# ototoi/pbrt-r3

Measured on AMD Instinct MI355X. Metric: Mrays/s, higher is better.
Workload: dtype f32

## Files before the change

### pbrt-r3_amd/csrc/pt_kernels.hip

```cpp
#include <hip/hip_runtime.h>
#include <cstdlib>
#include "pt_device.h"
#include "pt_device_math.h"
#include "pt_bxdf.h"
#include "pt_sphere.h"
#include "pt_quadric.h"
#include "pt_texture.h"
#include <type_traits>
#include "pt_lobes.h"
#include "pt_kernels.h"
#include "../../include/pbrtgpu.h"

#if PT_QUADRIC
#define PT_KERNEL __global__
namespace ptq {
#else
#define PT_KERNEL extern "C" __global__
#endif

#ifndef PT_SHADE_PF_DEEP
#define PT_SHADE_PF_DEEP 0
#endif
#ifndef PT_LOBES_IN_LDS
#define PT_LOBES_IN_LDS 1
// ... 1859 lines not shown
    const float span = cdf1 - cdf0;
    if (span > 0.0f) du /= span;
    *pdf = func_int > 0.0f ? func[idx] / func_int : 0.0f;
    *off = idx;
    return ((float)idx + du) * (1.0f / (float)n);
}
PT_DEV float spherical_theta_dev(V3 v) { return pt_acosf(clampf(v.z, -1.0f, 1.0f)); }
PT_DEV float spherical_phi_dev(V3 v) { const float p = pt_atan2f(v.y, v.x); return p < 0.0f ? p + 2.0f * PT_PI : p; }
#define PT_INV_2PI (PT_INV_PI * 0.5f)
PT_DEV bool env_sample_li(const PtScene& sc, const PtEnvLight& e, V2 u, V3* li, V3* wi, float* pdf) {
    float pdf0, pdf1;
    uint32_t v, u_off;
    const float d1 = dist1d_sample_continuous(e.mfunc, e.mcdf, e.nv, e.m_int, u.y, &pdf1, &v);
    const float d0 = dist1d_sample_continuous(e.func + (size_t)v * e.nu, e.cdf + (size_t)v * (e.nu + 1u), e.nu, e.mfunc[v], u.x, &pdf0, &u_off);
    const float map_pdf = pdf0 * pdf1;
    if (map_pdf <= 0.0f) return false;
    const float theta = d1 * PT_PI, phi = d0 * 2.0f * PT_PI;
    float sin_t, cos_t, sin_p, cos_p;
    pt_sincosf(theta, &sin_t, &cos_t);
    pt_sincosf(phi, &sin_p, &cos_p);
    sin_t = clampf(sin_t, 0.0f, 1.0f);
    *wi = sph_vector(e.l2w, mk3(sin_t * cos_p, sin_t * sin_p, cos_t));
    *pdf = sin_t == 0.0f ? 0.0f : map_pdf / (2.0f * PT_PI * PT_PI * sin_t);
    *li = env_lookup0(sc, e, mk2(d0, d1));
    return true;
}
PT_DEV uint32_t dist_cell(float x, uint32_t n) { return !(x > 0.0f) ? 0u : (x >= (float)n ? n - 1u : min((uint32_t)x, n - 1u)); }
PT_DEV float env_pdf_li(const PtEnvLight& e, V3 w) {
    const V3 wl = sph_vector(e.w2l, w);
    const float theta = spherical_theta_dev(wl), phi = spherical_phi_dev(wl);
    float sin_t, cos_t;
    pt_sincosf(theta, &sin_t, &cos_t);
    sin_t = clampf(sin_t, 0.0f, 1.0f);
    if (sin_t == 0.0f) return 0.0f;
    const uint32_t iu = dist_cell(phi * PT_INV_2PI * (float)e.nu, e.nu), iv = dist_cell(theta * PT_INV_PI * (float)e.nv, e.nv);
    return e.func[(size_t)iv * e.nu + iu] / e.m_int / (2.0f * PT_PI * PT_PI * sin_t);
}
PT_DEV V3 env_le(const PtScene& sc, const PtEnvLight& e, V3 d) {
    const V3 w = normalize(sph_vector(e.w2l, d));
    return env_lookup0(sc, e, mk2(spherical_phi_dev(w) * PT_INV_2PI, spherical_theta_dev(w) * PT_INV_PI));
}
PT_DEV V3 env_le_all(const PtScene& sc, V3 d) {
    V3 r = mk3(0.0f, 0.0f, 0.0f);
    for (uint32_t k = 0; k < sc.n_envs; k++) r = r + env_le(sc, scene_envs(sc)[k], d);
    return r;
}
PT_DEV float spot_falloff(const PtDeltaLight& dl, V3 w) {
    const V3 wl = normalize(mk3(dl.w2l[0] * w.x + dl.w2l[1] * w.y + dl.w2l[2] * w.z, dl.w2l[3] * w.x + dl.w2l[4] * w.y + dl.w2l[5] * w.z,
                                dl.w2l[6] * w.x + dl.w2l[7] * w.y + dl.w2l[8] * w.z));
    const float cos_theta = wl.z;
    if (cos_theta < dl.cos_total_width) return 0.0f;
    if (cos_theta >= dl.cos_falloff_start) return 1.0f;
    const float delta = (cos_theta - dl.cos_total_width) / (dl.cos_falloff_start - dl.cos_total_width);
    return (delta * delta) * (delta * delta);
}
PT_DEV void delta_sample_li(const PtDeltaLight& dl, V3 ref_p, V3* li, V3* wi, float* pdf, V3* lp) {
    const V3 v = ld3(dl.v), sp = ld3(dl.spectrum);
    *pdf = 1.0f;
    if (dl.kind == PT_DELTA_DISTANT) {
        *wi = v;
        *li = sp;
        *lp = ref_p + v * (2.0f * dl.radius);
        return;
    }
    *wi = normalize(v - ref_p);
    const float d2 = distance_squared(v, ref_p);
    if (dl.kind == PT_DELTA_SPOT) *li = sp * (spot_falloff(dl, -*wi) / d2);
    else *li = sp / d2;
    *lp = v;
}
template <bool DELTA>
PT_DEV bool light_is_delta(const PtLight& l) { if constexpr (DELTA) return (l.mesh_flags & PT_LIGHT_DELTA) != 0; else return false; }
template <bool SPH, bool ENV, bool DELTA = ENV>
PT_DEV bool light_sample_kind(const PtScene& sc, const PtLight& l, V3 ref_p, V3 ref_pe, V3 ref_n, V2 u, V3* li, V3* wi, float* pdf, V3* lp, V3* lperr,
                              V3* ln) {
    if constexpr (ENV) {
        if (l.mesh_flags & PT_LIGHT_INFINITE) {
            const PtEnvLight& e = scene_envs(sc)[__float_as_uint(l.p0[0])];
            if (!env_sample_li(sc, e, u, li, wi, pdf)) return false;
            *lp = ref_p + *wi * (2.0f * e.radius);
            *lperr = mk3(0.0f, 0.0f, 0.0f); *ln = mk3(0.0f, 0.0f, 0.0f);
            return true;
        }
        if constexpr (DELTA) {
            if (l.mesh_flags & PT_LIGHT_DELTA) {
                delta_sample_li(scene_deltas(sc)[__float_as_uint(l.p0[0])], ref_p, li, wi, pdf, lp);
                *lperr = mk3(0.0f, 0.0f, 0.0f); *ln = mk3(0.0f, 0.0f, 0.0f);
                return true;
            }
        }
    }
    return light_sample_any<SPH>(sc, l, ref_p, ref_pe, ref_n, u, li, wi, pdf, lp, lperr, ln);
}

PT_DEV const float* grid_lookup(const PtLightGrid& g, V3 p) {
    if (g.single) return g.data;
    uint32_t pi[3];
    float pc[3] = {p.x, p.y, p.z};
    for (int i = 0; i < 3; i++) {
        float o = pc[i] - g.wb_min[i];
        if (g.wb_max[i] > g.wb_min[i]) o = o / (g.wb_max[i] - g.wb_min[i]);
        o = clampf(o, 0.0f, 1.0f);
        float f = o * (float)g.voxels[i];
        uint32_t v = f > 0.0f ? (uint32_t)f : 0u;
        if (v > g.voxels[i] - 1) v = g.voxels[i] - 1;
        pi[i] = v;
    }
    size_t vox = ((size_t)pi[2] * g.voxels[1] + pi[1]) * g.voxels[0] + pi[0];
    if (g.row_of) vox = (size_t)(uint32_t)g.row_of[vox];
    return g.data + vox * g.stride;
}
PT_DEV uint32_t sample_discrete(const float* tab, uint32_t n, float u, float* pdf) {
    uint32_t idx;
    float f_idx, func_int;
    if (n <= 3) {
        const float4* q = reinterpret_cast<const float4*>(tab);
        float4 a = q[0], b = q[1];
        auto get = [&](uint32_t i) -> float {
            float lo = i == 0 ? a.x : (i == 1 ? a.y : (i == 2 ? a.z : a.w));
            float hi = i == 4 ? b.x : (i == 5 ? b.y : (i == 6 ? b.z : b.w));
            return i < 4 ? lo : hi;
        };
        uint32_t first = 0, len = n + 1;
        while (len > 0) {
            uint32_t half = len >> 1, middle = first + half;
            if (get(n + middle) <= u) { first = middle + 1; len -= half + 1; }
            else len = half;
        }
        idx = first == 0 ? 0 : first - 1;
        if (idx > n - 1) idx = n - 1;
        f_idx = get(idx);
        func_int = get(2 * n + 1);
    } else {
        const float* cdf = tab + n;
        uint32_t first = 0, len = n + 1;
        while (len > 0) {
            uint32_t half = len >> 1, middle = first + half;
            if (cdf[middle] <= u) { first = middle + 1; len -= half + 1; }
            else len = half;
        }
        idx = first == 0 ? 0 : first - 1;
        if (idx > n - 1) idx = n - 1;
        f_idx = tab[idx];
        func_int = tab[2 * n + 1];
    }
    *pdf = func_int > 0.0f ? f_idx * (1.0f / (float)n) / func_int : 0.0f;
    return idx;
}

PT_KERNEL void __launch_bounds__(PT_BLOCK) k_nee_resolve(PtScene sc, PtPaths P, PtQueues Q) {
    const uint32_t n = Q.counts[PT_Q_NEE];
    for (uint32_t i = blockIdx.x * blockDim.x + threadIdx.x; i < n; i += gridDim.x * blockDim.x) {
        const uint32_t p = Q.nee[i];
        const uint32_t nee = P.nee[p];
        const float4 A = P.pendA[p];
        V3 ld = mk3(0.0f, 0.0f, 0.0f);
        if ((nee & PT_NEE_SHADOW) && P.occluded[p] == 0) ld = ld + mk3(A.x, A.y, A.z);
        if (nee & PT_NEE_PROBE) {
            const int32_t best = P.probe_rec[p];
            if (best >= 0 && (uint32_t)best == sc.lights[nee >> 8].tri_rec) { float4 B = P.pendB[p]; ld = ld + mk3(B.x, B.y, B.z); }
        }
        V3 ldn = ld / A.w;
        float4 pb = P.pbeta[p];
        float4 L = P.L[p];
        V3 add = mk3(pb.x, pb.y, pb.z) * ldn;
        L.x += add.x; L.y += add.y; L.z += add.z;
        P.L[p] = L;
    }
}
PT_KERNEL void __launch_bounds__(PT_BLOCK) k_nee_resolve_env(PtScene sc, PtPaths P, PtQueues Q) {
    const uint32_t n = Q.counts[PT_Q_NEE];
    for (uint32_t i = blockIdx.x * blockDim.x + threadIdx.x; i < n; i += gridDim.x * blockDim.x) {
        const uint32_t p = Q.nee[i];
        const uint32_t nee = P.nee[p];
        const float4 A = P.pendA[p];
        V3 ld = mk3(0.0f, 0.0f, 0.0f);
        if ((nee & PT_NEE_SHADOW) && P.occluded[p] == 0) ld = ld + mk3(A.x, A.y, A.z);
        if (nee & PT_NEE_PROBE) {
            const int32_t best = P.probe_rec[p];
            const PtLight& lt = sc.lights[nee >> 8];
            const bool take = (lt.mesh_flags & PT_LIGHT_INFINITE) ? best < 0 : (best >= 0 && (uint32_t)best == lt.tri_rec);
            if (take) { float4 B = P.pendB[p]; ld = ld + mk3(B.x, B.y, B.z); }
        }
        V3 ldn = ld / A.w;
        float4 pb = P.pbeta[p];
        float4 L = P.L[p];
        V3 add = mk3(pb.x, pb.y, pb.z) * ldn;
        L.x += add.x; L.y += add.y; L.z += add.z;
        P.L[p] = L;
    }
}

PT_DEV uint32_t path_sort_bin(const PtScene& sc, const PtPaths& P, uint32_t p) {
    int32_t rec = P.hit_rec[p];
    if (rec < 0) return 0xffffffffu;
    uint32_t m1 = sc.tris[rec].flags >> PT_TRI_MATERIAL_SHIFT;
    return m1 == 0 ? (sc.n_instances ? PT_SORT_GENERAL0 : 0u) : sc.materials[m1 - 1].sort_bin;
}
PT_DEV uint32_t wave_bin_reserve(uint32_t* counters, uint32_t bin, bool valid) {
    uint32_t slot = 0;
    unsigned long long todo = __ballot(valid);
    const uint32_t lane = threadIdx.x & 63;
    while (todo) {
        int leader = __ffsll((long long)todo) - 1;
        uint32_t b0 = (uint32_t)__shfl((int)bin, leader, 64);
        unsigned long long same = __ballot(valid && bin == b0) & todo;
        uint32_t base = 0;
        if ((int)lane == leader) base = atomicAdd(&counters[b0], (uint32_t)__popcll(same));
        base = (uint32_t)__shfl((int)base, leader, 64);
        if (valid && bin == b0) slot = base + (uint32_t)__popcll(same & ((lane == 0) ? 0ull : (~0ull >> (64 - lane))));
        todo &= ~same;
    }
    return slot;
}
PT_DEV void sort_chunk(uint32_t n, uint32_t* lo, uint32_t* hi) {
    uint32_t chunk = (n + gridDim.x - 1) / gridDim.x;
    chunk = (chunk + 63u) & ~63u;
    *lo = min(n, blockIdx.x * chunk);
    *hi = min(n, *lo + chunk);
}
PT_KERNEL void __launch_bounds__(PT_BLOCK) k_sort_count(PtScene sc, PtPaths P, PtQueues Q) {
    __shared__ uint32_t s_cnt[PT_SORT_BINS];
    s_cnt[threadIdx.x] = 0;
    __syncthreads();
    uint32_t lo, hi;
    sort_chunk(Q.counts[PT_Q_CUR], &lo, &hi);
    for (uint32_t i = lo + threadIdx.x; i < ((hi + 63u) & ~63u); i += blockDim.x) {
        bool valid = i < hi;
        uint32_t bin = valid ? path_sort_bin(sc, P, Q.cur[i]) : 0xffffffffu;
        if (valid && Q.bin) Q.bin[i] = (uint16_t)bin;
        valid = valid && bin != 0xffffffffu;
        (void)wave_bin_reserve(s_cnt, valid ? bin : 0u, valid);
    }
    __syncthreads();
    uint32_t c = s_cnt[threadIdx.x];
    if (c) atomicAdd(&Q.counts[PT_SORT_COUNT0 + threadIdx.x], c);
}
PT_KERNEL void k_sort_scan(PtQueues Q) {
    __shared__ uint32_t s[PT_SORT_BINS];
    const uint32_t t = threadIdx.x;
    uint32_t c = Q.counts[PT_SORT_COUNT0 + t];
    s[t] = c;
    __syncthreads();
    for (uint32_t d = 1; d < PT_SORT_BINS; d <<= 1) {
        uint32_t v = t >= d ? s[t - d] : 0u;
        __syncthreads();
        s[t] += v;
        __syncthreads();
    }
    uint32_t excl = s[t] - c;
    Q.counts[PT_SORT_CURSOR0 + t] = excl;
    Q.counts[PT_SORT_COUNT0 + t] = 0;
    if (t == PT_SORT_GENERAL0) Q.counts[PT_Q_MATTE_END] = excl;
    if (t == PT_SORT_TEX0) Q.counts[PT_Q_TEX_BEGIN] = excl;
    if (t == PT_SORT_BINS - 1) Q.counts[PT_Q_GENERAL_END] = s[t];
}
PT_KERNEL void __launch_bounds__(PT_BLOCK) k_sort_scatter(PtScene sc, PtPaths P, PtQueues Q) {
    __shared__ uint32_t s_cnt[PT_SORT_BINS];
    s_cnt[threadIdx.x] = 0;
    __syncthreads();
    uint32_t lo, hi;
    sort_chunk(Q.counts[PT_Q_CUR], &lo, &hi);
    const uint32_t hi_round = (hi + 63u) & ~63u;
    auto bin_of = [&](uint32_t i, uint32_t p) -> uint32_t {
        if (Q.bin) { const uint32_t b = Q.bin[i]; return b == 0xffffu ? 0xffffffffu : b; }
        return path_sort_bin(sc, P, p);
    };
    for (uint32_t i = lo + threadIdx.x; i < hi_round; i += blockDim.x) {
        bool valid = i < hi;
        uint32_t bin = valid ? bin_of(i, Q.bin ? 0u : Q.cur[i]) : 0xffffffffu;
        valid = valid && bin != 0xffffffffu;
        (void)wave_bin_reserve(s_cnt, valid ? bin : 0u, valid);
    }
    __syncthreads();
    {
        uint32_t c = s_cnt[threadIdx.x];
        s_cnt[threadIdx.x] = c ? atomicAdd(&Q.counts[PT_SORT_CURSOR0 + threadIdx.x], c) : 0u;
    }
    __syncthreads();
    for (uint32_t i = lo + threadIdx.x; i < hi_round; i += blockDim.x) {
        bool valid = i < hi;
        uint32_t p = valid ? Q.cur[i] : 0u;
        uint32_t bin = valid ? bin_of(i, p) : 0xffffffffu;
        valid = valid && bin != 0xffffffffu;
        uint32_t pos = wave_bin_reserve(s_cnt, valid ? bin : 0u, valid);
        if (valid) Q.sorted[pos] = p;
    }
}

#ifndef PT_LOCAL_CHUNK
#define PT_LOCAL_CHUNK 4096u
#endif
PT_KERNEL void __launch_bounds__(PT_BLOCK) k_sort_local(PtScene sc, PtPaths P, PtQueues Q) {
    __shared__ uint32_t s_cnt[PT_SORT_BINS + 1];
    __shared__ uint32_t s_p[PT_LOCAL_CHUNK];
    __shared__ uint16_t s_b[PT_LOCAL_CHUNK];
    const uint32_t n = Q.counts[PT_Q_CUR];
    const uint32_t n_runs = (n + PT_LOCAL_CHUNK - 1u) / PT_LOCAL_CHUNK;
    for (uint32_t run = blockIdx.x; run < n_runs; run += gridDim.x) {
        const uint32_t lo = run * PT_LOCAL_CHUNK, len = min(PT_LOCAL_CHUNK, n - lo);
        for (uint32_t k = threadIdx.x; k <= PT_SORT_BINS; k += blockDim.x) s_cnt[k] = 0;
        __syncthreads();
        for (uint32_t i = threadIdx.x; i < len; i += blockDim.x) {
            const uint32_t p = Q.cur[lo + i];
            const uint32_t bin = path_sort_bin(sc, P, p);
            const uint32_t b = bin == 0xffffffffu ? PT_SORT_BINS : bin;
            s_p[i] = p; s_b[i] = (uint16_t)b;
            atomicAdd(&s_cnt[b], 1u);
        }
        __syncthreads();
        if (threadIdx.x == 0) {
            uint32_t acc = 0;
            for (uint32_t k = 0; k <= PT_SORT_BINS; k++) { const uint32_t c = s_cnt[k]; s_cnt[k] = acc; acc += c; }
        }
        __syncthreads();
        for (uint32_t i = threadIdx.x; i < len; i += blockDim.x) {
            const uint32_t pos = atomicAdd(&s_cnt[s_b[i]], 1u);
            Q.sorted[lo + pos] = s_p[i];
        }
        __syncthreads();
    }
}

#ifndef PT_SHADE_TICKET
#define PT_SHADE_TICKET 4
#endif
#ifndef PT_SHADE_FLUSH
#define PT_SHADE_FLUSH 4
// ... 103 lines not shown
            V3 c_n = n0, c_dpdu = dpdu0;
            textured_lobes(sc, mj, th, &tm, n, uv, &c_n, &c_dpdu, sh_dpdv, sh_dndu, sh_dndv);
            lm = &tm;
        }
        if (j == 0) eta0 = lm->bsdf_eta;
        if (lm->has_bsdf)
            for (uint32_t i = 0; i < lm->n_lobes && nl < PT_MIX_MAX_LOBES; i++) {
                mh->lobes[nl] = lm->lobes[i];
                mh->scales.lobe_leaf[nl] = j;
                nl++;
            }
        const uint32_t nc = mx.scales.n_chain[j];
        mh->scales.n_chain[j] = nc;
        for (uint32_t c = 0; c < nc; c++) {
            const uint32_t e = mx.chain[j][c], node = e & 0xffu, side = (e >> 8) & 1u;
            for (int q = 0; q < 3; q++) mh->scales.s[j][c][q] = ns[node][side][q];
        }
    }
    out->type = PT_MATERIAL_MIX;
    out->has_bsdf = 1; out->nonspecular = 0; out->spec_mask = 0; out->bsdf_eta = eta0;
    out->n_lobes = nl;
    for (uint32_t i = 0; i < nl; i++) {
        const uint32_t t = mh->lobes[i].type;
        if (!(t & kSpecular)) out->nonspecular++;
        if ((t & (kRefl | kSpecular)) == t) out->spec_mask |= 1u;
        if ((t & (kTrans | kSpecular)) == t) out->spec_mask |= 2u;
    }
}
PT_DEV void mix_hit(const PtScene& sc, int32_t material, const TexHit& th, PtMaterial* out, PtMixHit* mh, Surf& s) {
    const int32_t m0 = material_mix(sc, sc.materials[material]).leaf_material[0];
    const V3 n0 = s.sh_n, dpdu0 = s.sh_dpdu;
    uint32_t leaf0_done = 0;
    if (sc.materials[m0].textured) {
        textured_lobes(sc, m0, th, out, s.n, s.uv, &s.sh_n, &s.sh_dpdu, s.sh_dpdv, s.sh_dndu, s.sh_dndv);
        leaf0_done = 1;
    }
    mix_hit_lobes(sc, material, th, out, leaf0_done, mh, s.n, s.uv, n0, dpdu0, s.sh_dpdv, s.sh_dndu, s.sh_dndv);
}
PT_DEV uint32_t ray_sort_key(const PtScene& sc, V3 o, V3 d) {
    const float fx = (o.x - sc.wb_min[0]) * sc.cell_scale[0], fy = (o.y - sc.wb_min[1]) * sc.cell_scale[1], fz = (o.z - sc.wb_min[2]) * sc.cell_scale[2];
    const float top = (float)((1u << PT_SORT_CELL_BITS) - 1u);
    uint32_t cx = (uint32_t)fminf(fmaxf(fx, 0.0f), top), cy = (uint32_t)fminf(fmaxf(fy, 0.0f), top), cz = (uint32_t)fminf(fmaxf(fz, 0.0f), top);
    uint32_t m = 0;
#pragma unroll
    for (uint32_t b = 0; b < (uint32_t)PT_SORT_CELL_BITS; b++) m |= (((cx >> b) & 1u) | (((cy >> b) & 1u) << 1) | (((cz >> b) & 1u) << 2)) << (3u * b);
    return m | ((d.x < 0.0f ? 1u : 0u) | (d.y < 0.0f ? 2u : 0u) | (d.z < 0.0f ? 4u : 0u)) << (3u * PT_SORT_CELL_BITS);
}
#ifdef PT_PROFILE_SHADE
__device__ unsigned long long g_shade_prof[16];
#define PT_SHP(k) do { const unsigned long long t_now_ = (unsigned long long)__builtin_readcyclecounter(); shp_acc[k] += t_now_ - shp_last; shp_last = t_now_; } while (0)
#define PT_SHP_SYNC(k) do { asm volatile("s_waitcnt vmcnt(0)" ::: "memory"); PT_SHP(k); } while (0)
#else
#define PT_SHP(k) do { } while (0)
#define PT_SHP_SYNC(k) do { } while (0)
#endif
PT_DEV float opaque_zero() { float z = 0.0f; asm volatile("" : "+v"(z)); return z; }
template <bool GENERAL, bool SPH, bool TEX = false, bool INST = false, bool RES = false, int PART = 0, bool ENV = false, bool DELTA = false, bool MIX = false>
PT_DEV void shade_body(const PtScene& sc, const PtPaths& P, const PtQueues& Q, PtCounters* cnt, const uint32_t* list, uint32_t begin, uint32_t end,
                       uint32_t* ticket) {
    __shared__ unsigned long long s_vert;
    __shared__ float4 s_stage[PART == 2 ? 1 : 7][PT_BLOCK];
    __shared__ uint32_t s_pend[PT_SHADE_FLUSH][PT_BLOCK];
#if PT_LOBES_IN_LDS
    __shared__ uint32_t s_lobes[GENERAL ? PT_BLOCK / 64 : 1][PT_MAX_LOBES * (sizeof(PtLobe) / 4)];
#endif
    __shared__ uint32_t s_pkey[PT_SHADE_FLUSH][PT_BLOCK];
    if (threadIdx.x == 0) s_vert = 0;
#if PT_LIGHTS_IN_LDS
    __shared__ PtLight s_lights[PT_LIGHTS_IN_LDS];
    const bool lights_lds = sc.n_lights <= (uint32_t)PT_LIGHTS_IN_LDS && PART != 2;
    if (lights_lds) {
        const uint32_t nd = sc.n_lights * (uint32_t)(sizeof(PtLight) / 4);
        const uint32_t* src = reinterpret_cast<const uint32_t*>(sc.lights);
        uint32_t* dst = reinterpret_cast<uint32_t*>(s_lights);
        for (uint32_t k = threadIdx.x; k < nd; k += PT_BLOCK) dst[k] = src[k];
    }
#endif
    __syncthreads();
    uint32_t n_vert = 0;
    const uint32_t lane = threadIdx.x & 63;
    uint32_t chunk_left = 0, next_base = 0;
#ifdef PT_PROFILE_SHADE
    unsigned long long shp_acc[16] = {0, 0, 0, 0, 0, 0, 0, 0, 0, 0, 0, 0, 0, 0, 0, 0};
    unsigned long long shp_last = (unsigned long long)__builtin_readcyclecounter();
#endif
    uint32_t n_batch = 0, pend_want = 0;
    uint32_t pf_p = 0;
    int32_t pf_rec = -1;
    uint32_t pf_st = 0, pf_pk = 0;
    uint64_t pf_idx = 0;
    bool pf_valid = false;
    constexpr bool DEEP = PT_SHADE_PF_DEEP && !GENERAL && !SPH && !INST && PART == 0;
    float4 pf_ro = make_float4(0.0f, 0.0f, 0.0f, 0.0f), pf_rd = pf_ro, pf_beta = pf_ro, pf_ra = pf_ro, pf_rb = pf_ro, pf_rc = pf_ro;
    const unsigned long long below = (lane == 0) ? 0ull : (~0ull >> (64 - lane));
    auto flush_batch = [&]() {
        if (n_batch == 0) return;
        uint32_t tc = 0, tn = 0, ts = 0, tp = 0;
#pragma unroll
        for (uint32_t j = 0; j < PT_SHADE_FLUSH; j++) {
            if (j < n_batch) {
                const uint32_t e = pend_want >> (4u * j);
                tc += (uint32_t)__popcll(__ballot((e & 1u) != 0)); tn += (uint32_t)__popcll(__ballot((e & 2u) != 0));
                ts += (uint32_t)__popcll(__ballot((e & 4u) != 0)); tp += (uint32_t)__popcll(__ballot((e & 8u) != 0));
            }
        }
        uint32_t bc = 0, bn = 0, bs = 0, bp = 0;
        if (lane == 0) {
            if (tc) bc = atomicAdd(&Q.counts[PT_Q_NEXT], tc);
            if (tn) bn = atomicAdd(&Q.counts[PT_Q_NEE], tn);
            if (ts) bs = atomicAdd(&Q.counts[PT_Q_SHADOW], ts);
            if (tp) bp = atomicAdd(&Q.counts[PT_Q_PROBE], tp);
        }
        bc = (uint32_t)__builtin_amdgcn_readfirstlane((int)bc); bn = (uint32_t)__builtin_amdgcn_readfirstlane((int)bn);
        bs = (uint32_t)__builtin_amdgcn_readfirstlane((int)bs); bp = (uint32_t)__builtin_amdgcn_readfirstlane((int)bp);
#pragma unroll
        for (uint32_t j = 0; j < PT_SHADE_FLUSH; j++) {
            if (j < n_batch) {
                const uint32_t e = pend_want >> (4u * j), ep = s_pend[j][threadIdx.x];
                const unsigned long long mc = __ballot((e & 1u) != 0), mn = __ballot((e & 2u) != 0), ms = __ballot((e & 4u) != 0), mp = __ballot((e & 8u) != 0);
                if (e & 1u) Q.next[bc + (uint32_t)__popcll(mc & below)] = ep;
                if (e & 2u) Q.nee[bn + (uint32_t)__popcll(mn & below)] = ep;
                if (e & 4u) {
                    Q.shadow[bs + (uint32_t)__popcll(ms & below)] = ep;
                    if (Q.shadow_key) Q.shadow_key[bs + (uint32_t)__popcll(ms & below)] = s_pkey[j][threadIdx.x];
                }
                if (e & 8u) Q.probe[bp + (uint32_t)__popcll(mp & below)] = ep;
                bc += (uint32_t)__popcll(mc); bn += (uint32_t)__popcll(mn); bs += (uint32_t)__popcll(ms); bp += (uint32_t)__popcll(mp);
            }
        }
        n_batch = 0; pend_want = 0;
    };
    for (;;) {
        PT_SHP(11);
        if (chunk_left == 0) {
            uint32_t t0 = 0;
            if (lane == 0) t0 = atomicAdd(ticket, 64u * PT_SHADE_TICKET);
            next_base = begin + (uint32_t)__builtin_amdgcn_readfirstlane((int)t0);
            chunk_left = PT_SHADE_TICKET;
        }
        uint32_t base = next_base;
        next_base += 64u; chunk_left--;
        if (base >= end) break;
#ifdef PT_PROFILE_SHADE
        shp_acc[12]++;
#endif
        uint32_t item = base + lane;
        bool active = item < end;
        bool cont = false, want_nee = false, want_sh = false, want_pr = false;
        uint32_t p = 0;
        uint32_t wr = 0, o_nee = 0, o_state = 0;
        float4 o_ray_o = make_float4(0.0f, 0.0f, 0.0f, 0.0f), o_ray_d = o_ray_o, o_beta = o_ray_o;
        auto commit = [&]() {
            if constexpr (PART != 2) {
                if (wr & 4u) { P.sh_o[p] = s_stage[0][threadIdx.x]; P.sh_d[p] = s_stage[1][threadIdx.x]; }
                if (wr & 8u) { P.pr_o[p] = s_stage[2][threadIdx.x]; P.pr_d[p] = s_stage[3][threadIdx.x]; }
                if (wr & 16u) { P.pendA[p] = s_stage[4][threadIdx.x]; P.pendB[p] = s_stage[5][threadIdx.x]; P.pbeta[p] = s_stage[6][threadIdx.x]; P.nee[p] = o_nee; }
            }
            if (wr & 1u) P.ray_o[p] = o_ray_o;
            if (wr & 2u) { P.ray_d[p] = o_ray_d; P.beta[p] = o_beta; }
            if (wr & 32u) P.state[p] = o_state;
            wr = 0;
        };
#ifndef PT_DEFER_WIDE
#define PT_DEFER_WIDE 0
#endif
#ifndef PT_DEFER_SITES
#define PT_DEFER_SITES (PT_DEFER_WIDE ? 63 : 0)
#endif
#define PT_COMMIT_NOW(site) do { if constexpr ((TEX || INST) && !((PT_DEFER_SITES >> (site)) & 1)) commit(); } while (0)
        const bool had_pf = pf_valid;
        const uint32_t pf_p_now = pf_p;
        const int32_t pf_rec_now = pf_rec;
        const uint32_t pf_st_now = pf_st, pf_pk_now = pf_pk;
        const uint64_t pf_idx_now = pf_idx;
        const float4 pf_ro_now = pf_ro, pf_rd_now = pf_rd, pf_beta_now = pf_beta, pf_ra_now = pf_ra, pf_rb_now = pf_rb, pf_rc_now = pf_rc;
        pf_valid = chunk_left > 0;
        const bool pf_lane = pf_valid && next_base + lane < end;
        if (pf_lane) pf_p = list[next_base + lane];
        if (active) {
            p = had_pf ? pf_p_now : list[item];
            PT_SHP_SYNC(13);
            float4 ro4, rd4, beta4;
            if (DEEP && had_pf) { ro4 = pf_ro_now; rd4 = pf_rd_now; beta4 = pf_beta_now; }
            else { ro4 = P.ray_o[p]; rd4 = P.ray_d[p]; beta4 = P.beta[p]; }
            V3 ro = f4_3(ro4), rd = f4_3(rd4);
            int32_t rec = had_pf ? pf_rec_now : P.hit_rec[p];
            uint32_t st = had_pf ? pf_st_now : P.state[p];
            uint32_t dim = st & 0xffffu, bounces = (st >> 16) & 0xffu, flags = st >> 24;
            V3 beta = f4_3(beta4);
            float eta_scale = beta4.w;
            PT_SHP_SYNC(14);
            float4 rec_a = make_float4(0.0f, 0.0f, 0.0f, 0.0f), rec_b = rec_a, rec_c = rec_a;
            if (DEEP && had_pf) { rec_a = pf_ra_now; rec_b = pf_rb_now; rec_c = pf_rc_now; }
            else if (rec >= 0) {
                const float4* q = reinterpret_cast<const float4*>(sc.tris) + (size_t)(uint32_t)rec * 3;
                rec_a = q[0]; rec_b = q[1]; rec_c = q[2];
            }
            SamplerPre sm;
            sm.s.index = 0; sm.s.dim = dim; sm.s.px = 0; sm.s.py = 0; sm.dim0 = dim; sm.have = false;
            if (rec >= 0 && (int32_t)bounces < sc.max_depth) {
                sm.s.index = had_pf ? pf_idx_now : P.sobol_index[p];
                const uint32_t pk = had_pf ? pf_pk_now : P.pixel[p];
                sm.s.px = (int32_t)(pk & 0xffffu) + sc.film.sample_bounds[0];
                sm.s.py = (int32_t)(pk >> 16) + sc.film.sample_bounds[1];
                PT_SHP_SYNC(15);
                sm.begin(sc);
                PT_SHP_SYNC(10);
            }
            Surf s;
            float thit;
            bool found;
            if constexpr (INST) found = rec >= 0 && make_surf_inst<SPH>(sc, ro, rd, (uint32_t)rec, P.hit_inst[p], s, &thit);
            else found = rec >= 0 && make_surf_any_rec<SPH>(sc, ro, rd, (uint32_t)rec, rec_a, rec_b, rec_c, s, &thit);
            PT_SHP(0);
            if (pf_lane) {
                pf_rec = P.hit_rec[pf_p];
                pf_st = P.state[pf_p]; pf_idx = P.sobol_index[pf_p]; pf_pk = P.pixel[pf_p];
                if constexpr (DEEP) { pf_ro = P.ray_o[pf_p]; pf_rd = P.ray_d[pf_p]; pf_beta = P.beta[pf_p]; }
            }
            if constexpr (ENV && PART != 1) {
                if (rec < 0 && (bounces == 0 || (flags & PT_ST_SPECULAR))) {
                    float4 L = P.L[p];
                    for (uint32_t k = 0; k < sc.n_envs; k++) {
                        const V3 add = beta * env_le(sc, scene_envs(sc)[k], rd);
                        L.x += add.x; L.y += add.y; L.z += add.z;
                    }
                    P.L[p] = L;
                }
            }
            if (PART != 1 && found && (bounces == 0 || (flags & PT_ST_SPECULAR))) {
                int32_t li = s.light;
                if (li >= 0) {
                    V3 le = light_L(sc.lights[li], s.n, -rd);
                    float4 L = P.L[p];
                    V3 add = beta * le;
                    L.x += add.x; L.y += add.y; L.z += add.z;
                    P.L[p] = L;
                }
            }
            if (found && (int32_t)bounces < sc.max_depth) {
                bool no_bsdf = s.material < 0;
                PtMaterial tm;
                std::conditional_t<MIX, PtMixHit, PtNoMix> mh;
                bool use_tm = false;
                if constexpr (TEX) {
                    if (!no_bsdf && sc.materials[s.material].textured) {
                        TexHit th;
                        th.p = s.p; th.uv = s.uv;
                        RayDiffs rdf;
                        const bool has_diff = (flags & PT_ST_CAMERA) != 0;
                        if (has_diff) {
                            Sampler sl;
                            sl.index = P.sobol_index[p];
                            sl.dim = 2;
                            uint32_t pk2 = P.pixel[p];
                            sl.px = (int32_t)(pk2 & 0xffffu) + sc.film.sample_bounds[0];
                            sl.py = (int32_t)(pk2 >> 16) + sc.film.sample_bounds[1];
                            V2 u_lens = mk2(0.0f, 0.0f);
                            if (sc.cam.lens_radius > 0.0f) u_lens = sl.get_2d(sc);
                            float2 pf = P.p_film[p];
                            camera_differentials(sc, mk2(pf.x, pf.y), u_lens, ro, rd, rdf);
                        }
                        compute_differentials(th, s.p, s.n, s.dpdu, s.dpdv, has_diff, rdf);
                        if constexpr (MIX) {
                            if (sc.materials[s.material].mix1) mix_hit(sc, s.material, th, &tm, &mh, s);
                            else textured_lobes(sc, s.material, th, &tm, s.n, s.uv, &s.sh_n, &s.sh_dpdu, s.sh_dpdv, s.sh_dndu, s.sh_dndv);
                        } else
                        textured_lobes(sc, s.material, th, &tm, s.n, s.uv, &s.sh_n, &s.sh_dpdu, s.sh_dpdv, s.sh_dndu, s.sh_dndv);
                        use_tm = true;
                        no_bsdf = tm.has_bsdf == 0;
                    }
                }
                if constexpr (RES) {
                    if (!no_bsdf && sc.materials[s.material].textured) {
                        const float4* r = P.tex_res + (size_t)p * PT_TEX_RES_F4;
                        const float4 r0 = r[0], r1 = r[1], r2 = r[2], r3 = r[3], r4 = r[4], r5 = r[5], r6 = r[6], r7 = r[7], r8 = r[8];
                        PtMatParams mp = sc.mat_params[s.material];
                        mp.m.kd[0] = r0.x; mp.m.kd[1] = r0.y; mp.m.kd[2] = r0.z; mp.m.ks[0] = r0.w; mp.m.ks[1] = r1.x; mp.m.ks[2] = r1.y;
                        mp.m.kr[0] = r1.z; mp.m.kr[1] = r1.w; mp.m.kr[2] = r2.x; mp.m.kt[0] = r2.y; mp.m.kt[1] = r2.z; mp.m.kt[2] = r2.w;
                        mp.m.opacity[0] = r3.x; mp.m.opacity[1] = r3.y; mp.m.opacity[2] = r3.z; mp.m.sigma = r3.w;
                        mp.m.metal_eta[0] = r4.x; mp.m.metal_eta[1] = r4.y; mp.m.metal_eta[2] = r4.z; mp.m.metal_k[0] = r4.w; mp.m.metal_k[1] = r5.x; mp.m.metal_k[2] = r5.y;
                        mp.m.uroughness = r5.z; mp.m.vroughness = r5.w; mp.m.eta = r6.x;
                        build_lobes_call(mp.m, r6.y, r6.z, r6.w, tm);
                        s.sh_n = mk3(r7.x, r7.y, r7.z); s.sh_dpdu = mk3(r7.w, r8.x, r8.y);
                        use_tm = true;
                        no_bsdf = tm.has_bsdf == 0;
                    }
                }
                if constexpr (GENERAL) { if (!no_bsdf && !use_tm) no_bsdf = sc.materials[s.material].has_bsdf == 0; }
                if (no_bsdf) {
                    if constexpr (PART != 1) {
                        V3 no = offset_ray_origin(s.p, s.p_error, s.n, rd);
                        o_ray_o = make_float4(no.x, no.y, no.z, PT_INF); wr |= 1u;
                        cont = true; PT_COMMIT_NOW(0);
                    }
                } else {
                    if constexpr (PART != 1) n_vert++;
                    Bsdf b;
                    std::conditional_t<MIX, MBsdf, GBsdf> gb;
                    bool nonspecular;
                    float bsdf_eta = 1.0f;
                    if constexpr (GENERAL) {
                        const PtMaterial& m = use_tm ? tm : sc.materials[s.material];
                        gb.ns = s.sh_n; gb.ng = s.n;
                        gb.ss = normalize(s.sh_dpdu);
                        gb.ts = normalize(cross(gb.ns, gb.ss));
                        gb.lobes = m.lobes; gb.n_lobes = m.n_lobes;
                        if constexpr (MIX) {
                            gb.scales = nullptr;
                            if (sc.materials[s.material].mix1) {
                                if (use_tm) { gb.lobes = mh.lobes; gb.scales = &mh.scales; }
                                else { const PtMix& mx = material_mix(sc, sc.materials[s.material]); gb.lobes = mx.lobes; gb.n_lobes = mx.n_lobes; gb.scales = &mx.scales; }
                            }
                        }
#if PT_LOBES_IN_LDS
                        if constexpr (!INST && !TEX) {
                            const int32_t mat0 = __builtin_amdgcn_readfirstlane(s.material);
                            const unsigned long long here = __ballot(1);
                            if (__ballot(use_tm || s.material != mat0) == 0ull) {
                                const uint32_t nd = (uint32_t)__builtin_amdgcn_readfirstlane((int)m.n_lobes) * (uint32_t)(sizeof(PtLobe) / 4);
                                const uint32_t nact = (uint32_t)__popcll(here), rank = (uint32_t)__popcll(here & below);
                                const uint32_t* src = reinterpret_cast<const uint32_t*>(sc.materials[mat0].lobes);
                                uint32_t* dst = &s_lobes[threadIdx.x >> 6][0];
                                for (uint32_t k = rank; k < nd; k += nact) dst[k] = src[k];
                                __builtin_amdgcn_fence(__ATOMIC_RELEASE, "wavefront");
                                __builtin_amdgcn_wave_barrier();
                                __builtin_amdgcn_fence(__ATOMIC_ACQUIRE, "wavefront");
                                gb.lobes = reinterpret_cast<const PtLobe*>(dst);
                            }
                        }
#endif
                        nonspecular = m.nonspecular > 0;
                        bsdf_eta = m.bsdf_eta;
                    } else {
                        const PtMaterial& m = sc.materials[s.material];
                        b.ns = s.sh_n; b.ng = s.n;
                        b.ss = normalize(s.sh_dpdu);
                        b.ts = normalize(cross(b.ns, b.ss));
                        b.r = mk3(m.kd[0], m.kd[1], m.kd[2]);
                        b.n_lobes = is_black(b.r) ? 0 : 1;
                        b.oren = clampf(m.sigma, 0.0f, 90.0f) != 0.0f;
                        b.oa = m.oren_a; b.ob = m.oren_b;
                        nonspecular = b.n_lobes > 0;
                    }
                    const uint32_t kNoSpec = PT_BSDF_ALL & ~PT_BSDF_SPECULAR;
                    auto eval_f = [&](V3 wo_w, V3 wi_w) -> V3 {
                        if constexpr (MIX) return mbsdf_f(gb, wo_w, wi_w, kNoSpec);
                        else if constexpr (GENERAL) return gbsdf_f(gb, wo_w, wi_w, kNoSpec); else return bsdf_f(b, wo_w, wi_w);
                    };
                    auto eval_pdf = [&](V3 wo_w, V3 wi_w) -> float {
                        if constexpr (MIX) return mbsdf_pdf(gb, wo_w, wi_w, kNoSpec);
                        else if constexpr (GENERAL) return gbsdf_pdf(gb, wo_w, wi_w, kNoSpec); else return bsdf_pdf(b, wo_w, wi_w);
                    };
                    auto sample_bsdf = [&](V3 wo_w, V2 uu, uint32_t fl, V3* f_o, V3* wi_o, float* pdf_o, uint32_t* type_o) -> bool {
                        if constexpr (MIX) return mbsdf_sample_f(gb, wo_w, uu, fl, f_o, wi_o, pdf_o, type_o);
                        else if constexpr (GENERAL) return gbsdf_sample_f(gb, wo_w, uu, fl, f_o, wi_o, pdf_o, type_o);
                        else { *type_o = PT_BSDF_REFLECTION | PT_BSDF_DIFFUSE; return bsdf_sample_f(b, wo_w, uu, f_o, wi_o, pdf_o); }
                    };
                    PT_SHP(1);
                    if constexpr (PART == 2) {
                        if (nonspecular && sc.n_lights > 0) sm.s.dim += (P.nee[p] & PT_NEE_DIMS5) ? 5u : 1u;
                    }
                    if (PART != 2 && nonspecular && sc.n_lights > 0) {
                        const float* tab = grid_lookup(sc.grid, s.p);
                        float light_pdf;
                        uint32_t light_num = sample_discrete(tab, sc.n_lights, sm.get_1d(sc), &light_pdf);
                        PT_SHP(2);
                        if (light_pdf > 0.0f) {
                            V2 u_light = sm.get_2d(sc);
                            V2 u_scat = sm.get_2d(sc);
                            PT_SHP(3);
#if PT_LIGHTS_IN_LDS
                            const PtLight& lt = lights_lds ? s_lights[light_num] : sc.lights[light_num];
#else
                            const PtLight& lt = sc.lights[light_num];
#endif
                            uint32_t nee = (light_num << 8) | (PART == 1 ? PT_NEE_DIMS5 : 0u);
                            V3 A = mk3(0.0f, 0.0f, 0.0f), B = mk3(0.0f, 0.0f, 0.0f);
                            V3 li, wi, lp, lperr, ln;
                            float lpdf;
                            bool sampled;
                            if constexpr (ENV) sampled = light_sample_kind<SPH, true, DELTA>(sc, lt, s.p, s.p_error, s.n, u_light, &li, &wi, &lpdf, &lp, &lperr, &ln);
                            else sampled = light_sample_any<SPH>(sc, lt, s.p, s.p_error, s.n, u_light, &li, &wi, &lpdf, &lp, &lperr, &ln);
                            if (sampled) {
                                if (lpdf > 0.0f && !is_black(li)) {
                                    V3 f = eval_f(s.wo, wi) * abs_dot(wi, s.sh_n);
                                    float spdf = eval_pdf(s.wo, wi);
                                    if (!is_black(f)) {
                                        V3 origin = offset_ray_origin(s.p, s.p_error, s.n, lp - s.p);
                                        V3 target = offset_ray_origin(lp, lperr, ln, origin - lp);
                                        V3 sd = target - origin;
                                        s_stage[0][threadIdx.x] = make_float4(origin.x, origin.y, origin.z, 1.0f - PT_SHADOW_EPS);
                                        s_stage[1][threadIdx.x] = make_float4(sd.x, sd.y, sd.z, 0.0f);
                                        if (Q.shadow_key) s_pkey[n_batch][threadIdx.x] = ray_sort_key(sc, origin, sd);
                                        wr |= 4u; PT_COMMIT_NOW(1);
                                        if (light_is_delta<DELTA>(lt)) A = f * li / lpdf;
                                        else {
                                            float weight = power_heuristic(lpdf, spdf);
                                            A = f * li * (weight / lpdf);
                                        }
                                        nee |= PT_NEE_SHADOW;
                                    }
                                }
                            }
                            PT_SHP(4);
                            V3 f2, wi2;
                            float spdf2;
                            uint32_t type2;
                            if (!light_is_delta<DELTA>(lt) && sample_bsdf(s.wo, u_scat, kNoSpec, &f2, &wi2, &spdf2, &type2)) {
                                V3 f = f2 * abs_dot(wi2, s.sh_n);
                                if (!is_black(f) && spdf2 > 0.0f) {
                                    V3 po = offset_ray_origin(s.p, s.p_error, s.n, wi2);
                                    bool env_done = false;
                                    if constexpr (ENV) {
                                        if (lt.mesh_flags & PT_LIGHT_INFINITE) {
                                            env_done = true;
                                            const PtEnvLight& e = scene_envs(sc)[__float_as_uint(lt.p0[0])];
                                            const float lp2 = env_pdf_li(e, wi2);
                                            if (lp2 != 0.0f) {
                                                const float weight = power_heuristic(spdf2, lp2);
                                                const V3 le = env_le(sc, e, wi2);
                                                B = f * le * 1.0f * (weight / spdf2);
                                                s_stage[2][threadIdx.x] = make_float4(po.x, po.y, po.z, PT_INF);
                                                s_stage[3][threadIdx.x] = make_float4(wi2.x, wi2.y, wi2.z, 0.0f);
                                                wr |= 8u; PT_COMMIT_NOW(2);
                                                nee |= PT_NEE_PROBE;
                                            }
                                        }
                                    }
                                    if (!env_done) {
                                    Surf ls;
                                    float lt_t;
                                    bool lhit;
                                    if (lt.mesh_flags & (PT_MESH_HAS_N | PT_MESH_HAS_S | PT_MESH_HAS_UV | PT_LIGHT_SPHERE)) {
                                        lhit = make_surf_any<SPH>(sc, po, wi2, lt.tri_rec, ls, &lt_t);
                                    } else {
                                        TriVerts ltv;
                                        ltv.p0 = ld3(lt.p0); ltv.p1 = ld3(lt.p1); ltv.p2 = ld3(lt.p2);
                                        ltv.prim = lt.prim;
                                        ltv.flags = ((lt.mesh_flags & PT_MESH_TWO_SIDED) ? 0u : PT_TRI_ONE_SIDED) |
                                                    ((((lt.mesh_flags & PT_MESH_REVERSE_ORIENTATION) != 0) ^ ((lt.mesh_flags & PT_MESH_SWAPS_HANDEDNESS) != 0)) ? PT_TRI_FLIP : 0u);
                                        lhit = make_surf_tv(sc, po, wi2, ltv, 0u, ls, &lt_t);
                                    }
                                    if (lhit) {
                                        float lp2 = distance_squared(s.p, ls.p) / (abs_dot(ls.n, -wi2) * lt.area);
                                        if (isinf(lp2)) lp2 = 0.0f;
                                        if (lp2 != 0.0f) {
                                            float weight = power_heuristic(spdf2, lp2);
                                            V3 le = light_L(lt, ls.n, -wi2);
                                            B = f * le * 1.0f * (weight / spdf2);
                                            s_stage[2][threadIdx.x] = make_float4(po.x, po.y, po.z, PT_INF);
                                            s_stage[3][threadIdx.x] = make_float4(wi2.x, wi2.y, wi2.z, 0.0f);
                                            wr |= 8u; PT_COMMIT_NOW(2);
                                            nee |= PT_NEE_PROBE;
                                        }
                                    }
                                    }
                                }
                            }
                            PT_SHP(5);
                            if (nee & (PT_NEE_SHADOW | PT_NEE_PROBE)) {
                                s_stage[4][threadIdx.x] = make_float4(A.x, A.y, A.z, light_pdf);
                                s_stage[5][threadIdx.x] = make_float4(B.x, B.y, B.z, 0.0f);
                                s_stage[6][threadIdx.x] = make_float4(beta.x, beta.y, beta.z, 0.0f);
                                o_nee = nee; wr |= 16u; PT_COMMIT_NOW(3);
                                want_nee = true;
                                want_sh = (nee & PT_NEE_SHADOW) != 0;
                                want_pr = (nee & PT_NEE_PROBE) != 0;
                            } else if constexpr (PART == 1) { P.nee[p] = nee; }
                        } else if constexpr (PART == 1) { P.nee[p] = 0u; }
                    }
                    PT_SHP(6);
                    if constexpr (PART != 1) {
                    V2 u = sm.get_2d(sc);
                    PT_SHP(7);
                    V3 f, wi;
                    float pdf;
                    uint32_t stype;
                    const V3 wo_ray = -rd;
                    if (sample_bsdf(wo_ray, u, PT_BSDF_ALL, &f, &wi, &pdf, &stype) && !(is_black(f) || pdf == 0.0f)) {
                        beta = beta * (f * (abs_dot(wi, s.sh_n) / pdf));
                        if (stype & PT_BSDF_SPECULAR) flags |= PT_ST_SPECULAR; else flags &= ~PT_ST_SPECULAR;
                        if ((stype & PT_BSDF_SPECULAR) && (stype & PT_BSDF_TRANSMISSION))
                            eta_scale *= dot(wo_ray, s.n) > 0.0f ? bsdf_eta * bsdf_eta : 1.0f / (bsdf_eta * bsdf_eta);
                        V3 no = offset_ray_origin(s.p, s.p_error, s.n, wi);
                        bool alive = true;
                        V3 rr = beta * eta_scale;
                        float mx = max3(rr.x, rr.y, rr.z);
                        if (mx < sc.rr_threshold && bounces > 3) {
                            float q = fmaxf(0.05f, 1.0f - mx);
                            if (sm.get_1d(sc) < q) alive = false;
                            else beta = beta / (1.0f - q);
                        }
                        if (alive) {
                            o_ray_o = make_float4(no.x, no.y, no.z, PT_INF);
                            o_ray_d = make_float4(wi.x, wi.y, wi.z, opaque_zero());
                            o_beta = make_float4(beta.x, beta.y, beta.z, eta_scale);
                            wr |= 3u; PT_COMMIT_NOW(4);
                            bounces++;
                            cont = true;
                        }
                    }
                    }
                    dim = sm.s.dim;
                }
                if (cont) { o_state = (dim & 0xffffu) | ((bounces & 0xffu) << 16) | ((flags & ~PT_ST_CAMERA) << 24); wr |= 32u; } PT_COMMIT_NOW(5);
            }
        }
        if constexpr (DEEP) {
            if (pf_lane && pf_rec >= 0) {
                const float4* q = reinterpret_cast<const float4*>(sc.tris) + (size_t)(uint32_t)pf_rec * 3;
                pf_ra = q[0]; pf_rb = q[1]; pf_rc = q[2];
            }
        }
        PT_SHP(8);
        commit();
        s_pend[n_batch][threadIdx.x] = p;
        pend_want |= ((cont ? 1u : 0u) | (want_nee ? 2u : 0u) | (want_sh ? 4u : 0u) | (want_pr ? 8u : 0u)) << (4u * n_batch);
        if (++n_batch == PT_SHADE_FLUSH) flush_batch();
        PT_SHP(9);
    }
    flush_batch();
#ifdef PT_PROFILE_SHADE
    if (lane == 0) { for (int k = 0; k < 16; k++) atomicAdd(&g_shade_prof[k], shp_acc[k]); }
#endif
    if (n_vert) atomicAdd(&s_vert, (unsigned long long)n_vert);
    __syncthreads();
    if (threadIdx.x == 0 && s_vert) atomicAdd(&cnt->vertices, s_vert);
}
PT_KERNEL void __launch_bounds__(PT_BLOCK, PT_SHADE_WAVES) k_shade(PtScene sc, PtPaths P, PtQueues Q, PtCounters* cnt) {
    shade_body<false, false>(sc, P, Q, cnt, Q.cur, 0u, Q.counts[PT_Q_CUR], &Q.counts[PT_Q_TICKET]);
}
PT_KERNEL void __launch_bounds__(PT_BLOCK, PT_SHADE_WAVES) k_shade_matte_sorted(PtScene sc, PtPaths P, PtQueues Q, PtCounters* cnt) {
    shade_body<false, false>(sc, P, Q, cnt, Q.sorted, 0u, Q.counts[PT_Q_MATTE_END], &Q.counts[PT_Q_TICKET]);
}
PT_KERNEL void __launch_bounds__(PT_BLOCK, PT_SHADE_GEN_WAVES) k_shade_general(PtScene sc, PtPaths P, PtQueues Q, PtCounters* cnt) {
    shade_body<true, false>(sc, P, Q, cnt, Q.sorted, Q.counts[PT_Q_MATTE_END], Q.counts[PT_Q_TEX_BEGIN], &Q.counts[PT_Q_TICKET2]);
}
PT_KERNEL void __launch_bounds__(PT_BLOCK, PT_WIDE_KERNEL_WAVES) k_shade_matte_sorted_sph(PtScene sc, PtPaths P, PtQueues Q, PtCounters* cnt) {
    shade_body<false, true>(sc, P, Q, cnt, Q.sorted, 0u, Q.counts[PT_Q_MATTE_END], &Q.counts[PT_Q_TICKET]);
}
PT_KERNEL void __launch_bounds__(PT_BLOCK, PT_WIDE_KERNEL_WAVES) k_shade_general_sph(PtScene sc, PtPaths P, PtQueues Q, PtCounters* cnt) {
    shade_body<true, true>(sc, P, Q, cnt, Q.sorted, Q.counts[PT_Q_MATTE_END], Q.counts[PT_Q_TEX_BEGIN], &Q.counts[PT_Q_TICKET2]);
}
PT_KERNEL void __launch_bounds__(PT_BLOCK, PT_WIDE_KERNEL_WAVES) k_shade_general_inst(PtScene sc, PtPaths P, PtQueues Q, PtCounters* cnt) {
    shade_body<true, true, true, true>(sc, P, Q, cnt, Q.sorted, Q.counts[PT_Q_MATTE_END], Q.counts[PT_Q_GENERAL_END], &Q.counts[PT_Q_TICKET2]);
}
PT_KERNEL void __launch_bounds__(PT_BLOCK, PT_WIDE_KERNEL_WAVES) k_shade_general_inst_plain(PtScene sc, PtPaths P, PtQueues Q, PtCounters* cnt) {
    shade_body<true, false, false, true>(sc, P, Q, cnt, Q.sorted, Q.counts[PT_Q_MATTE_END], Q.counts[PT_Q_GENERAL_END], &Q.counts[PT_Q_TICKET2]);
}
PT_KERNEL void __launch_bounds__(PT_BLOCK, PT_SHADE_TEX_WAVES) k_shade_general_tex(PtScene sc, PtPaths P, PtQueues Q, PtCounters* cnt) {
    shade_body<true, true, true>(sc, P, Q, cnt, Q.sorted, Q.counts[PT_Q_TEX_BEGIN], Q.counts[PT_Q_GENERAL_END], &Q.counts[PT_Q_TICKET3]);
}

template <bool SPH, bool ALL = false>
PT_DEV void tex_resolve_body(const PtScene& sc, const PtPaths& P, const PtQueues& Q) {
    const uint32_t begin = ALL ? 0u : Q.counts[PT_Q_TEX_BEGIN], end = ALL ? Q.counts[PT_Q_CUR] : Q.counts[PT_Q_GENERAL_END];
    const uint32_t* list = ALL ? Q.cur : Q.sorted;
    __shared__ float s_texval[3 * PT_TEX_PROG_MAX][PT_BLOCK];
    for (uint32_t i = begin + blockIdx.x * blockDim.x + threadIdx.x; i < end; i += gridDim.x * blockDim.x) {
        const uint32_t p = list[i];
        const int32_t rec = P.hit_rec[p];
        if constexpr (ALL) {
            if (rec < 0) continue;
            const uint32_t m1 = sc.tris[rec].flags >> PT_TRI_MATERIAL_SHIFT;
            if (m1 == 0u || !sc.materials[m1 - 1u].textured) continue;
        }
        const uint32_t st = P.state[p];
        const uint32_t bounces = (st >> 16) & 0xffu, flags = st >> 24;
        if (rec < 0 || (int32_t)bounces >= sc.max_depth) continue;
        const float4 ro4 = P.ray_o[p], rd4 = P.ray_d[p];
        const V3 ro = f4_3(ro4), rd = f4_3(rd4);
        const float4* q = reinterpret_cast<const float4*>(sc.tris) + (size_t)(uint32_t)rec * 3;
        const float4 rec_a = q[0], rec_b = q[1], rec_c = q[2];
        Surf s;
        float thit;
        if (!make_surf_any_rec<SPH>(sc, ro, rd, (uint32_t)rec, rec_a, rec_b, rec_c, s, &thit)) continue;
        if (s.material < 0 || !sc.materials[s.material].textured) continue;
        TexHit th;
        th.p = s.p; th.uv = s.uv;
        RayDiffs rdf;
        const bool has_diff = (flags & PT_ST_CAMERA) != 0;
        if (has_diff) {
            Sampler sl;
            sl.index = P.sobol_index[p];
            sl.dim = 2;
            const uint32_t pk2 = P.pixel[p];
            sl.px = (int32_t)(pk2 & 0xffffu) + sc.film.sample_bounds[0];
            sl.py = (int32_t)(pk2 >> 16) + sc.film.sample_bounds[1];
            V2 u_lens = mk2(0.0f, 0.0f);
            if (sc.cam.lens_radius > 0.0f) u_lens = sl.get_2d(sc);
            const float2 pf = P.p_film[p];
            camera_differentials(sc, mk2(pf.x, pf.y), u_lens, ro, rd, rdf);
        }
        compute_differentials(th, s.p, s.n, s.dpdu, s.dpdv, has_diff, rdf);
        PtMatParams mp;
        float a3[3];
        textured_params_t<true>(sc, s.material, th, mp, a3, s.n, s.uv, &s.sh_n, &s.sh_dpdu, s.sh_dpdv, s.sh_dndu, s.sh_dndv, &s_texval[0][threadIdx.x]);
        float4* o = P.tex_res + (size_t)p * PT_TEX_RES_F4;
        o[0] = make_float4(mp.m.kd[0], mp.m.kd[1], mp.m.kd[2], mp.m.ks[0]);
        o[1] = make_float4(mp.m.ks[1], mp.m.ks[2], mp.m.kr[0], mp.m.kr[1]);
        o[2] = make_float4(mp.m.kr[2], mp.m.kt[0], mp.m.kt[1], mp.m.kt[2]);
        o[3] = make_float4(mp.m.opacity[0], mp.m.opacity[1], mp.m.opacity[2], mp.m.sigma);
        o[4] = make_float4(mp.m.metal_eta[0], mp.m.metal_eta[1], mp.m.metal_eta[2], mp.m.metal_k[0]);
        o[5] = make_float4(mp.m.metal_k[1], mp.m.metal_k[2], mp.m.uroughness, mp.m.vroughness);
        o[6] = make_float4(mp.m.eta, a3[0], a3[1], a3[2]);
        o[7] = make_float4(s.sh_n.x, s.sh_n.y, s.sh_n.z, s.sh_dpdu.x);
        o[8] = make_float4(s.sh_dpdu.y, s.sh_dpdu.z, 0.0f, 0.0f);
    }
}
#ifndef PT_TEX_RESOLVE_WAVES
#define PT_TEX_RESOLVE_WAVES 2
#endif
PT_KERNEL void __launch_bounds__(PT_BLOCK, PT_TEX_RESOLVE_WAVES) k_tex_resolve(PtScene sc, PtPaths P, PtQueues Q) { tex_resolve_body<false>(sc, P, Q); }
PT_KERNEL void __launch_bounds__(PT_BLOCK, PT_TEX_RESOLVE_WAVES) k_tex_resolve_sph(PtScene sc, PtPaths P, PtQueues Q) { tex_resolve_body<true>(sc, P, Q); }
PT_KERNEL void __launch_bounds__(PT_BLOCK, PT_TEX_RESOLVE_WAVES) k_tex_resolve_all(PtScene sc, PtPaths P, PtQueues Q) { tex_resolve_body<false, true>(sc, P, Q); }
PT_KERNEL void __launch_bounds__(PT_BLOCK, PT_SHADE_GEN_WAVES) k_shade_all_res(PtScene sc, PtPaths P, PtQueues Q, PtCounters* cnt) {
    shade_body<true, false, false, false, true>(sc, P, Q, cnt, Q.cur, 0u, Q.counts[PT_Q_CUR], &Q.counts[PT_Q_TICKET]);
}
PT_KERNEL void __launch_bounds__(PT_BLOCK, PT_SHADE_GEN_WAVES) k_shade_general_res(PtScene sc, PtPaths P, PtQueues Q, PtCounters* cnt) {
    shade_body<true, false, false, false, true>(sc, P, Q, cnt, Q.sorted, Q.counts[PT_Q_TEX_BEGIN], Q.counts[PT_Q_GENERAL_END], &Q.counts[PT_Q_TICKET3]);
}
// ... 1464 lines not shown
```

Measured before the change: 1183.

## Pre-fold shadow-only NEE contribution in shade to shrink resolve traffic

```diff
diff --git a/pbrt-r3_amd/csrc/pt_kernels.hip b/pbrt-r3_amd/csrc/pt_kernels.hip
--- a/pbrt-r3_amd/csrc/pt_kernels.hip
+++ b/pbrt-r3_amd/csrc/pt_kernels.hip
@@ -2035,8 +2035,16 @@
     const uint32_t n = Q.counts[PT_Q_NEE];
     for (uint32_t i = blockIdx.x * blockDim.x + threadIdx.x; i < n; i += gridDim.x * blockDim.x) {
         const uint32_t p = Q.nee[i];
+        const float4 A = P.pendA[p];
+        if (__float_as_uint(A.w) == 0u) {
+            if (P.occluded[p] == 0) {
+                float4 L = P.L[p];
+                L.x += A.x; L.y += A.y; L.z += A.z;
+                P.L[p] = L;
+            }
+            continue;
+        }
         const uint32_t nee = P.nee[p];
-        const float4 A = P.pendA[p];
         V3 ld = mk3(0.0f, 0.0f, 0.0f);
         if ((nee & PT_NEE_SHADOW) && P.occluded[p] == 0) ld = ld + mk3(A.x, A.y, A.z);
         if (nee & PT_NEE_PROBE) {
@@ -2055,8 +2063,16 @@
     const uint32_t n = Q.counts[PT_Q_NEE];
     for (uint32_t i = blockIdx.x * blockDim.x + threadIdx.x; i < n; i += gridDim.x * blockDim.x) {
         const uint32_t p = Q.nee[i];
+        const float4 A = P.pendA[p];
+        if (__float_as_uint(A.w) == 0u) {
+            if (P.occluded[p] == 0) {
+                float4 L = P.L[p];
+                L.x += A.x; L.y += A.y; L.z += A.z;
+                P.L[p] = L;
+            }
+            continue;
+        }
         const uint32_t nee = P.nee[p];
-        const float4 A = P.pendA[p];
         V3 ld = mk3(0.0f, 0.0f, 0.0f);
         if ((nee & PT_NEE_SHADOW) && P.occluded[p] == 0) ld = ld + mk3(A.x, A.y, A.z);
         if (nee & PT_NEE_PROBE) {
@@ -2466,6 +2482,7 @@
         float4 o_ray_o = make_float4(0.0f, 0.0f, 0.0f, 0.0f), o_ray_d = o_ray_o, o_beta = o_ray_o;
         auto commit = [&]() {
             if constexpr (PART != 2) {
+                if (wr & 64u) { P.pendA[p] = s_stage[4][threadIdx.x]; if constexpr (PART == 1) P.nee[p] = o_nee; }
                 if (wr & 4u) { P.sh_o[p] = s_stage[0][threadIdx.x]; P.sh_d[p] = s_stage[1][threadIdx.x]; }
                 if (wr & 8u) { P.pr_o[p] = s_stage[2][threadIdx.x]; P.pr_d[p] = s_stage[3][threadIdx.x]; }
                 if (wr & 16u) { P.pendA[p] = s_stage[4][threadIdx.x]; P.pendB[p] = s_stage[5][threadIdx.x]; P.pbeta[p] = s_stage[6][threadIdx.x]; P.nee[p] = o_nee; }
@@ -2684,11 +2701,7 @@
                             V2 u_light = sm.get_2d(sc);
                             V2 u_scat = sm.get_2d(sc);
                             PT_SHP(3);
-#if PT_LIGHTS_IN_LDS
-                            const PtLight& lt = lights_lds ? s_lights[light_num] : sc.lights[light_num];
-#else
-                            const PtLight& lt = sc.lights[light_num];
-#endif
+                            auto estimate = [&](const PtLight& lt) __attribute__((always_inline)) {
                             uint32_t nee = (light_num << 8) | (PART == 1 ? PT_NEE_DIMS5 : 0u);
                             V3 A = mk3(0.0f, 0.0f, 0.0f), B = mk3(0.0f, 0.0f, 0.0f);
                             V3 li, wi, lp, lperr, ln;
@@ -2773,7 +2786,18 @@
                                 }
                             }
                             PT_SHP(5);
-                            if (nee & (PT_NEE_SHADOW | PT_NEE_PROBE)) {
+                            bool folded = false;
+                            if ((nee & (PT_NEE_SHADOW | PT_NEE_PROBE)) == PT_NEE_SHADOW) {
+                                const V3 add = beta * ((mk3(0.0f, 0.0f, 0.0f) + A) / light_pdf);
+                                if (isfinite(beta.x) && isfinite(beta.y) && isfinite(beta.z) && isfinite(A.x) && isfinite(A.y) && isfinite(A.z) && isfinite(light_pdf)) {
+                                    s_stage[4][threadIdx.x] = make_float4(add.x, add.y, add.z, 0.0f);
+                                    o_nee = nee; wr |= 64u; PT_COMMIT_NOW(3);
+                                    want_nee = true; want_sh = true;
+                                    folded = true;
+                                }
+                            }
+                            if (folded) { }
+                            else if (nee & (PT_NEE_SHADOW | PT_NEE_PROBE)) {
                                 s_stage[4][threadIdx.x] = make_float4(A.x, A.y, A.z, light_pdf);
                                 s_stage[5][threadIdx.x] = make_float4(B.x, B.y, B.z, 0.0f);
                                 s_stage[6][threadIdx.x] = make_float4(beta.x, beta.y, beta.z, 0.0f);
@@ -2782,6 +2806,12 @@
                                 want_sh = (nee & PT_NEE_SHADOW) != 0;
                                 want_pr = (nee & PT_NEE_PROBE) != 0;
                             } else if constexpr (PART == 1) { P.nee[p] = nee; }
+                            };
+#if PT_LIGHTS_IN_LDS
+                            if (lights_lds) estimate(s_lights[light_num]); else estimate(sc.lights[light_num]);
+#else
+                            estimate(sc.lights[light_num]);
+#endif
                         } else if constexpr (PART == 1) { P.nee[p] = 0u; }
                     }
                     PT_SHP(6);
```

Result: faster. 1196, median of 6 (+1.1%).
